# Napoliee/Expressive-FastSpeech2-Mandarin

Hardware: AMD Instinct MI355X
Metric: mel-frames/sec/GPU (batch-64 synth) at 1/2/4/8 MI355X; RTF (higher is better)
Workload: dtype bf16; 1 GPU; cfg2: batch=64 x 64 phonemes per GPU, ESD-Chinese-Singing-MFA model.yaml, FastSpeech2.forward eval bf16; global_batch=64, seq_len=64, mel_frames_per_gpu_batch=24883, T_max=430, parallelism=dp1 (independent shards, no collective), hip_graph=True

## Files before the change

### expressive-fastspeech2-mandarin_amd/csrc/lr.hip

```cpp
#include <cstdlib>
#include <type_traits>

#include "fs2_common.h"
#include "fs2hip_prosody.h"

namespace {

constexpr int kScanThreads = 256;
constexpr int kLdsCum = 2048;

__device__ __forceinline__ int64_t frames_of(const void *dur, int kind, float d_control, const float *d_map,
                                             int64_t idx, float *d_rounded) {
  if (kind == FS2_DUR_I64) {
    int64_t d = reinterpret_cast<const int64_t *>(dur)[idx];
    return d > 0 ? d : 0;
  }
  float v = reinterpret_cast<const float *>(dur)[idx];
  if (kind == FS2_DUR_LOGPRED) {
    float r = rintf(expf(v) - 1.0f) * (d_map != nullptr ? d_map[idx] : d_control);
    r = r < 0.0f ? 0.0f : r;
    if (d_rounded) d_rounded[idx] = r;
    v = r;
  }
  if (!(v > 0.0f)) return 0;
  if (v >= 9.2e18f) return INT64_MAX / 4;
  return (int64_t)v;
}

__global__ __launch_bounds__(kScanThreads) void lr_durations_kernel(const void *dur, int kind, float d_control,
                                                                    const float *d_map, int L, int32_t *cum,
                                                                    int64_t *mel_len, float *d_rounded) {
  const int b = blockIdx.x;
  const int tid = threadIdx.x;
  const int lane = tid & 63, wid = tid >> 6;
  const int per = (L + kScanThreads - 1) / kScanThreads;
  const int i0 = min(tid * per, L), i1 = min(i0 + per, L);
  const int64_t base = (int64_t)b * L;

  int64_t local = 0;
  for (int i = i0; i < i1; ++i) local += frames_of(dur, kind, d_control, d_map, base + i, nullptr);

  int64_t incl = local;
#pragma unroll
  for (int o = 1; o < 64; o <<= 1) {
    int64_t y = __shfl_up(incl, o, 64);
    if (lane >= o) incl += y;
  }
  __shared__ int64_t wave_tot[kScanThreads / 64];
  if (lane == 63) wave_tot[wid] = incl;
  __syncthreads();
  int64_t prefix = 0;
  for (int w = 0; w < wid; ++w) prefix += wave_tot[w];
  int64_t run = prefix + incl - local;

  for (int i = i0; i < i1; ++i) {
    run += frames_of(dur, kind, d_control, d_map, base + i, d_rounded);
    cum[base + i] = (int32_t)(run < 0x7fffffff ? run : 0x7fffffff);
  }
  if (tid == kScanThreads - 1) {
    int64_t total = 0;
    for (int w = 0; w < kScanThreads / 64; ++w) total += wave_tot[w];
    mel_len[b] = total;
  }
}

template <typename TX, typename TO, bool HAS_PE, int ROWS, bool NT>
__global__ __launch_bounds__(256) void lr_expand_kernel(const TX *__restrict__ x, const int32_t *__restrict__ cum,
                                                        const int64_t *__restrict__ mel_len, int L, int D, int T_out,
                                                        const float *__restrict__ pe, TO *__restrict__ out,
                                                        int32_t *__restrict__ index_map,
                                                        const int32_t *__restrict__ out_cu) {
  constexpr int UNR = ROWS / 8;
  const int b = blockIdx.y;
  const int t0 = blockIdx.x * ROWS;
  const int tid = threadIdx.x;
  const int t_end = out_cu != nullptr ? min(T_out, out_cu[b + 1] - out_cu[b]) : T_out;
  if (t0 >= t_end && index_map == nullptr) return;
  __shared__ int src[ROWS];
  __shared__ int32_t scum[kLdsCum];
  const int64_t ml = mel_len[b];
  const int lim = (int)(ml < (int64_t)T_out ? ml : (int64_t)T_out);
  const int32_t *c = cum + (int64_t)b * L;
  const bool in_lds = L <= kLdsCum;
  if (in_lds)
    for (int i = tid; i < L; i += 256) scum[i] = c[i];
  __syncthreads();
  const int32_t *sc = in_lds ? scum : c;
  if (tid < ROWS) {
    const int t = t0 + tid;
    int s = -1;
    if (t < lim) {
      int lo = 0, hi = L - 1;
      while (lo < hi) {
        const int mid = (lo + hi) >> 1;
        if (sc[mid] > t) hi = mid; else lo = mid + 1;
      }
      s = lo;
    }
    src[tid] = s;
    if (index_map != nullptr && t < T_out) index_map[(int64_t)b * T_out + t] = s;
  }
  __syncthreads();
  if (out == nullptr) return;
  const int vpr = D >> 3;
  const int rows = min(ROWS, t_end - t0);
  if (rows <= 0) return;
  const int total = rows * vpr;
  const TX *xb = x + (int64_t)b * L * D;
  TO *ob = out + ((out_cu != nullptr ? (int64_t)out_cu[b] : (int64_t)b * T_out) + t0) * D;
  for (int base = tid; base < total; base += 256 * UNR) {
    float v[UNR][8];
#pragma unroll
    for (int u = 0; u < UNR; ++u) {
      const int e = base + u * 256;
      const int r = e / vpr;
      const int col = (e - r * vpr) << 3;
      const int s = e < total ? src[r] : -1;
      if (s >= 0) {
        load8(xb + (int64_t)s * D + col, v[u]);
      } else {
#pragma unroll
        for (int q = 0; q < 8; ++q) v[u][q] = 0.0f;
      }
      if constexpr (HAS_PE) {
        if (e < total) {
          float p[8];
          load8(pe + (int64_t)(t0 + r) * D + col, p);
#pragma unroll
          for (int q = 0; q < 8; ++q) v[u][q] += p[q];
        }
      }
    }
#pragma unroll
    for (int u = 0; u < UNR; ++u) {
      const int e = base + u * 256;
      if (e < total) {
        if constexpr (NT && sizeof(TO) == 2) {
          bf16x8 o;
#pragma unroll
          for (int q = 0; q < 8; ++q) o[q] = (bf16)v[u][q];
          __builtin_nontemporal_store(o, reinterpret_cast<bf16x8 *>(ob + (int64_t)e * 8));
        } else {
          store8(ob + (int64_t)e * 8, v[u]);
        }
      }
    }
  }
}

template <typename TX, typename TO, int ROWS, bool NT>
void launch_expand_v(const void *x, const int32_t *cum, const int64_t *mel_len, int B, int L, int D, int T_out,
                     const float *pe, void *out, int32_t *index_map, const int32_t *out_cu, hipStream_t s) {
  dim3 grid((T_out + ROWS - 1) / ROWS, B);
  if (pe != nullptr)
    hipLaunchKernelGGL((lr_expand_kernel<TX, TO, true, ROWS, NT>), grid, dim3(256), 0, s,
                       reinterpret_cast<const TX *>(x), cum, mel_len, L, D, T_out, pe, reinterpret_cast<TO *>(out),
                       index_map, out_cu);
  else
    hipLaunchKernelGGL((lr_expand_kernel<TX, TO, false, ROWS, NT>), grid, dim3(256), 0, s,
                       reinterpret_cast<const TX *>(x), cum, mel_len, L, D, T_out, pe, reinterpret_cast<TO *>(out),
                       index_map, out_cu);
}

template <typename TX, typename TO>
void launch_expand(const void *x, const int32_t *cum, const int64_t *mel_len, int B, int L, int D, int T_out,
                   const float *pe, void *out, int32_t *index_map, const int32_t *out_cu, hipStream_t s) {
  launch_expand_v<TX, TO, 32, true>(x, cum, mel_len, B, L, D, T_out, pe, out, index_map, out_cu, s);
}

__global__ __launch_bounds__(256) void lr_bwd_kernel(const float *__restrict__ dy, const int32_t *__restrict__ cum,
                                                     int L, int D, int T, float *__restrict__ dx) {
  constexpr int PH = 8;
  const int b = blockIdx.y, i0 = blockIdx.x * PH;
  const int vpr = D >> 3;
  const int32_t *c = cum + (int64_t)b * L;
  const float *db = dy + (int64_t)b * T * D;
  for (int e = threadIdx.x; e < PH * vpr; e += 256) {
    const int i = i0 + e / vpr;
    if (i >= L) break;
    const int col = (e - (i - i0) * vpr) << 3;
    const int t0 = i == 0 ? 0 : min(c[i - 1], T);
    const int t1 = min(c[i], T);
    float acc[8] = {0.f, 0.f, 0.f, 0.f, 0.f, 0.f, 0.f, 0.f};
    for (int t = t0; t < t1; ++t) {
      float v[8];
      load8(db + (int64_t)t * D + col, v);
#pragma unroll
      for (int q = 0; q < 8; ++q) acc[q] += v[q];
    }
    store8(dx + ((int64_t)b * L + i) * D + col, acc);
  }
}

struct LrFusedArgs {
  const void *x;
  const void *dur;
  int dur_kind;
  float d_control;
  const float *d_map;
  const int32_t *cum_in;
  const int64_t *mel_len_in;
  const int64_t *lens;
  int B, L, D, T;
  const float *pe;
  void *out;
  int32_t *cum;
  int64_t *mel_len;
  float *d_rounded;
  int32_t *cu;
  int2 *row_pos;
  int32_t *rowmap;
  int store;
  const float *proj_src;
  const float *proj_pe;
  int NP;
  bf16 *proj_out;
  int padded;
  int32_t *index_map;
};

template <typename TX, typename TO, bool HAS_PE, int ROWS>
__global__ __launch_bounds__(256) void lr_fused_kernel(LrFusedArgs a) {
  constexpr int UNR = ROWS / 8 < 8 ? ROWS / 8 : 8;
  const int b = blockIdx.y, t0 = blockIdx.x * ROWS;
  const int tid = threadIdx.x, lane = tid & 63, wv = tid >> 6;
  const int L = a.L, T = a.T, D = a.D;
  __shared__ int32_t scum[kLdsCum];
  __shared__ int src[ROWS];
  __shared__ int64_t wtot[4];
  __shared__ int32_t wcu[4];
  __shared__ int64_t s_ml;
  const bool first = blockIdx.x == 0;
  auto clen = [&](int j) {
    const int64_t l = a.lens[j];
    return (int32_t)(l < 0 ? 0 : (l > T ? T : l));
  };
  int32_t part = 0;
  if (!a.padded)
    for (int j = tid; j < b; j += 256) part += clen(j);

  if (a.dur != nullptr) {
    const int per = (L + 255) / 256;
    const int i0 = min(tid * per, L), i1 = min(i0 + per, L);
    const int64_t base = (int64_t)b * L;
    int64_t local = 0;
    for (int i = i0; i < i1; ++i) local += frames_of(a.dur, a.dur_kind, a.d_control, a.d_map, base + i, nullptr);
    int64_t incl = local;
#pragma unroll
    for (int o = 1; o < 64; o <<= 1) {
      const int64_t y = __shfl_up(incl, o, 64);
      if (lane >= o) incl += y;
    }
    if (lane == 63) wtot[wv] = incl;
    __syncthreads();
    int64_t run = incl - local;
    for (int w = 0; w < wv; ++w) run += wtot[w];
    for (int i = i0; i < i1; ++i) {
      run += frames_of(a.dur, a.dur_kind, a.d_control, a.d_map, base + i, first ? a.d_rounded : nullptr);
      const int32_t c = (int32_t)(run < 0x7fffffff ? run : 0x7fffffff);
      scum[i] = c;
      if (first) a.cum[base + i] = c;
    }
    if (tid == 0) {
      const int64_t total = (wtot[0] + wtot[1]) + (wtot[2] + wtot[3]);
      s_ml = total;
      if (first) a.mel_len[b] = total;
    }
  } else {
    const int32_t *c = a.cum_in + (int64_t)b * L;
    for (int i = tid; i < L; i += 256) scum[i] = c[i];
    if (tid == 0) s_ml = a.mel_len_in[b];
  }

#pragma unroll
  for (int o = 32; o > 0; o >>= 1) part += __shfl_xor(part, o, 64);
  if (lane == 0) wcu[wv] = part;
  __syncthreads();
  const int32_t cu_b = a.padded ? b * T : (wcu[0] + wcu[1]) + (wcu[2] + wcu[3]);
  const int32_t len_b = a.padded ? T : clen(b);
  if (first && tid == 0 && !a.padded) {
    a.cu[b] = cu_b;
    if (b == a.B - 1) a.cu[a.B] = cu_b + len_b;
  }

  const int64_t ml = s_ml;
  const int lim = (int)(ml < (int64_t)T ? ml : (int64_t)T);
  if (tid < ROWS) {
    const int t = t0 + tid;
    int sidx = -1;
    if (t < lim) {
      int lo = 0, hi = L - 1;
      while (lo < hi) {
        const int mid = (lo + hi) >> 1;
        if (scum[mid] > t) hi = mid; else lo = mid + 1;
      }
      sidx = lo;
    }
    src[tid] = sidx;
    if (a.index_map != nullptr && t < T) a.index_map[(int64_t)b * T + t] = sidx;
    if (t < T && !a.padded) {
      if (a.rowmap != nullptr) a.rowmap[(int64_t)b * T + t] = t < len_b ? cu_b + t : -1;
      if (a.row_pos != nullptr && t < len_b) a.row_pos[cu_b + t] = make_int2(t, len_b);
    }
  }
  __syncthreads();

  const int rows = min(ROWS, min(T, (int)len_b) - t0);
  if (rows <= 0) return;
  const int vpr = D >> 3, total = rows * vpr;
  const TX *xb = reinterpret_cast<const TX *>(a.x) + (int64_t)b * L * D;
  TO *ob = reinterpret_cast<TO *>(a.out) + ((int64_t)cu_b + t0) * D;
  const bool proj = a.proj_out != nullptr;
  auto gather = [&](auto UC, int me, int nthr) {
    constexpr int U = decltype(UC)::value;
    for (int base = me; base < total; base += nthr * U) {
      float v[U][8];
#pragma unroll
      for (int u = 0; u < U; ++u) {
        const int e = base + u * nthr;
        const int r = e / vpr;
        const int col = (e - r * vpr) << 3;
        const int sidx = e < total ? src[r] : -1;
        if (sidx >= 0) {
          load8(xb + (int64_t)sidx * D + col, v[u]);
        } else {
#pragma unroll
          for (int q = 0; q < 8; ++q) v[u][q] = 0.0f;
        }
        if constexpr (HAS_PE) {
          if (e < total) {
            float pv[8];
            load8(a.pe + (int64_t)(t0 + r) * D + col, pv);
#pragma unroll
            for (int q = 0; q < 8; ++q) v[u][q] += pv[q];
          }
        }
      }
#pragma unroll
      for (int u = 0; u < U; ++u) {
        const int e = base + u * nthr;
        if (e < total) {
          if constexpr (sizeof(TO) == 2) {
            bf16x8 o;
#pragma unroll
            for (int q = 0; q < 8; ++q) o[q] = (bf16)v[u][q];
            bf16x8 *dst = reinterpret_cast<bf16x8 *>(ob + (int64_t)e * 8);
            if (a.store == 0)
              __builtin_nontemporal_store(o, dst);
            else if (a.store == 1)
              *dst = o;
            else
              __builtin_amdgcn_raw_buffer_store_b128(__builtin_bit_cast(__attribute__((ext_vector_type(4))) unsigned, o),
                                                     __builtin_amdgcn_make_buffer_rsrc(dst, (short)0, 16, 0x00020000), 0u,
                                                     0, 16);
          } else {
            store8(ob + (int64_t)e * 8, v[u]);
          }
        }
      }
    }
  };
  gather(std::integral_constant<int, UNR>{}, tid, 256);
  if (proj && wv < 3) {
    constexpr int RB = 8;
    const int NP = a.NP, cg = NP >> 3;
    const float *tb = a.proj_pe + (int64_t)t0 * NP;
    const float *sb = a.proj_src + (int64_t)b * L * NP;
    bf16 *pb = a.proj_out + ((int64_t)cu_b + t0) * NP;
    const int lanes = 192 / cg * cg;
    if (tid < lanes) {
      const int c = (tid % cg) * 8, r1 = tid / cg, rs = lanes / cg;
      for (int r0 = r1; r0 < rows; r0 += RB * rs) {
        float4 tv[RB][2], sv[RB][2];
#pragma unroll
        for (int u = 0; u < RB; ++u) {
          const int r = min(r0 + u * rs, rows - 1);
          const int sidx = src[r];
          const float *tp = tb + (int64_t)r * NP + c;
          tv[u][0] = *reinterpret_cast<const float4 *>(tp);
          tv[u][1] = *reinterpret_cast<const float4 *>(tp + 4);
          if (sidx >= 0) {
            const float *sp = sb + (int64_t)sidx * NP + c;
            sv[u][0] = *reinterpret_cast<const float4 *>(sp);
            sv[u][1] = *reinterpret_cast<const float4 *>(sp + 4);
          } else {
            sv[u][0] = sv[u][1] = make_float4(0.f, 0.f, 0.f, 0.f);
          }
        }
#pragma unroll
        for (int u = 0; u < RB; ++u) {
          const int r = r0 + u * rs;
          if (r < rows) {
            const bf16x8 o{(bf16)(tv[u][0].x + sv[u][0].x), (bf16)(tv[u][0].y + sv[u][0].y),
                           (bf16)(tv[u][0].z + sv[u][0].z), (bf16)(tv[u][0].w + sv[u][0].w),
                           (bf16)(tv[u][1].x + sv[u][1].x), (bf16)(tv[u][1].y + sv[u][1].y),
                           (bf16)(tv[u][1].z + sv[u][1].z), (bf16)(tv[u][1].w + sv[u][1].w)};
            __builtin_nontemporal_store(o, reinterpret_cast<bf16x8 *>(pb + (int64_t)r * NP + c));
          }
        }
      }
    }
  }
}

__global__ __launch_bounds__(256) void length_mask_kernel(const int64_t *__restrict__ lens, int width, int64_t n,
                                                          bool *__restrict__ mask) {
  const int64_t i = (int64_t)blockIdx.x * 256 + threadIdx.x;
  if (i >= n) return;
  const int64_t b = i / width;
  mask[i] = (int64_t)(i - b * width) >= lens[b];
}

__global__ __launch_bounds__(256) void seq_cu_kernel(const int64_t *__restrict__ lens, int B, int T,
                                                     int32_t *__restrict__ cu) {
  __shared__ int32_t part[257];
  const int tid = threadIdx.x;
  const int per = (B + 255) / 256;
  const int i0 = min(tid * per, B), i1 = min(i0 + per, B);
  int32_t local = 0;
  for (int i = i0; i < i1; ++i) {
    const int64_t l = lens[i];
    local += (int32_t)(l < 0 ? 0 : (l > T ? T : l));
  }
  part[tid + 1] = local;
  if (tid == 0) part[0] = 0;
  __syncthreads();
  if (tid == 0)
    for (int i = 1; i <= 256; ++i) part[i] += part[i - 1];
  __syncthreads();
  int32_t run = part[tid];
  for (int i = i0; i < i1; ++i) {
    cu[i] = run;
    const int64_t l = lens[i];
    run += (int32_t)(l < 0 ? 0 : (l > T ? T : l));
  }
  if (tid == 255) cu[B] = part[256];
}

__global__ __launch_bounds__(256) void seq_rows_kernel(const int32_t *__restrict__ cu, int B, int T,
                                                       int2 *__restrict__ row_pos, int32_t *__restrict__ rowmap) {
  const int64_t i = (int64_t)blockIdx.x * 256 + threadIdx.x;
  if (i >= (int64_t)B * T) return;
  const int b = (int)(i / T), t = (int)(i - (int64_t)b * T);
  const int c = cu[b], len = cu[b + 1] - c;
  if (rowmap != nullptr) rowmap[i] = t < len ? c + t : -1;
  if (row_pos != nullptr && t < len) row_pos[c + t] = make_int2(t, len);
}

constexpr int kSeqMaxB = 4096;
__global__ __launch_bounds__(256) void seq_layout_kernel(const int64_t *__restrict__ lens, int B, int T,
                                                         int32_t *__restrict__ cu, int2 *__restrict__ row_pos,
                                                         int32_t *__restrict__ rowmap, int margin) {
  __shared__ int32_t scu[kSeqMaxB + 1];
  __shared__ int32_t wsum[4];
  const int tid = threadIdx.x, lane = tid & 63, wv = tid >> 6;
  const int per = (B + 255) / 256;
  const int i0 = min(tid * per, B), i1 = min(i0 + per, B);
  auto clen = [&](int i) {
    int64_t l = lens[i];
    if (margin > 0) l = l + 2 * (int64_t)margin > T ? T : l + margin;
    return (int32_t)(l < 0 ? 0 : (l > T ? T : l));
  };
  int32_t local = 0;
  for (int i = i0; i < i1; ++i) local += clen(i);
  int32_t v = local;
#pragma unroll
  for (int o = 1; o < 64; o <<= 1) {
    const int32_t u = __shfl_up(v, o);
    if (lane >= o) v += u;
  }
  if (lane == 63) wsum[wv] = v;
  __syncthreads();
  int32_t run = v - local;
  for (int w = 0; w < wv; ++w) run += wsum[w];
  for (int i = i0; i < i1; ++i) {
    scu[i] = run;
    run += clen(i);
  }
  if (tid == 0) scu[B] = wsum[0] + wsum[1] + wsum[2] + wsum[3];
  __syncthreads();
  if (blockIdx.x == 0)
    for (int i = tid; i <= B; i += 256) cu[i] = scu[i];
  const int64_t i = (int64_t)blockIdx.x * 256 + tid;
  if (i >= (int64_t)B * T) return;
  const int b = (int)(i / T), t = (int)(i - (int64_t)b * T);
  const int c = scu[b], len = scu[b + 1] - c;
  if (rowmap != nullptr) rowmap[i] = t < len ? c + t : -1;
  if (row_pos != nullptr && t < len) row_pos[c + t] = make_int2(t, len);
}

__global__ __launch_bounds__(256) void len_stats_kernel(const int64_t *__restrict__ lens, int B,
                                                        const int32_t *__restrict__ bad, int32_t *__restrict__ meta) {
  __shared__ int64_t smax[4], ssum[4];
  const int tid = threadIdx.x, lane = tid & 63, wv = tid >> 6;
  int64_t mx = 0, sm = 0;
  for (int i = tid; i < B; i += 256) {
    const int64_t l = lens[i] < 0 ? 0 : lens[i];
    mx = l > mx ? l : mx;
    sm += l;
  }
#pragma unroll
  for (int o = 32; o > 0; o >>= 1) {
    const int64_t a = __shfl_xor(mx, o), b = __shfl_xor(sm, o);
    mx = a > mx ? a : mx;
    sm += b;
  }
  if (lane == 0) {
    smax[wv] = mx;
    ssum[wv] = sm;
  }
  __syncthreads();
  if (tid == 0) {
    int64_t m = 0, t = 0;
    for (int w = 0; w < 4; ++w) {
      m = smax[w] > m ? smax[w] : m;
      t += ssum[w];
    }
    meta[0] = (int32_t)(m < 0x7fffffff ? m : 0x7fffffff);
    meta[1] = (int32_t)(t < 0x7fffffff ? t : 0x7fffffff);
    meta[2] = bad != nullptr ? *bad : 0;
  }
}

}

extern "C" int fs2_seq_layout_margin(const int64_t *lens, int B, int T, int margin, int32_t *cu, int32_t *row_pos,
                                     int32_t *rowmap, fs2_stream_t stream) {
  if (lens == nullptr || cu == nullptr || B < 0 || T < 0 || margin < 0 || B > kSeqMaxB ||
      (int64_t)B * T > 0x7fffff00LL)
    return FS2_EINVAL;
  const int64_t n = (int64_t)B * T;
  hipLaunchKernelGGL(seq_layout_kernel, dim3((unsigned)(n > 0 ? (n + 255) / 256 : 1)), dim3(256), 0, as_stream(stream),
                     lens, B, T, cu, reinterpret_cast<int2 *>(row_pos), rowmap, margin);
  FS2_CHECK_LAUNCH();
  return FS2_OK;
}

extern "C" int fs2_seq_layout(const int64_t *lens, int B, int T, int32_t *cu, int32_t *row_pos, int32_t *rowmap,
                              fs2_stream_t stream) {
  if (lens == nullptr || cu == nullptr || B < 0 || T < 0 || (int64_t)B * T > 0x7fffff00LL) return FS2_EINVAL;
  hipStream_t s = as_stream(stream);
  if (B <= kSeqMaxB) return fs2_seq_layout_margin(lens, B, T, 0, cu, row_pos, rowmap, stream);
  hipLaunchKernelGGL(seq_cu_kernel, dim3(1), dim3(256), 0, s, lens, B, T, cu);
  FS2_CHECK_LAUNCH();
  if ((rowmap != nullptr || row_pos != nullptr) && (int64_t)B * T > 0) {
    hipLaunchKernelGGL(seq_rows_kernel, dim3((unsigned)(((int64_t)B * T + 255) / 256)), dim3(256), 0, s, cu, B, T,
                       reinterpret_cast<int2 *>(row_pos), rowmap);
    FS2_CHECK_LAUNCH();
  }
  return FS2_OK;
}

extern "C" int fs2_length_masks(const int64_t *lens, int B, int width, bool *mask, fs2_stream_t stream) {
  if (lens == nullptr || mask == nullptr || B < 0 || width < 0) return FS2_EINVAL;
  const int64_t n = (int64_t)B * width;
  if (n == 0) return FS2_OK;
  hipLaunchKernelGGL(length_mask_kernel, dim3((unsigned)((n + 255) / 256)), dim3(256), 0, as_stream(stream), lens, width,
                     n, mask);
  FS2_CHECK_LAUNCH();
  return FS2_OK;
}

extern "C" int fs2_lr_durations_map(const void *dur, int dur_kind, float d_control, const float *d_map, int B, int L,
                                    int32_t *cum, int64_t *mel_len, float *d_rounded, fs2_stream_t stream) {
  if (dur == nullptr || cum == nullptr || mel_len == nullptr || B < 0 || L <= 0) return FS2_EINVAL;
  if (dur_kind < FS2_DUR_I64 || dur_kind > FS2_DUR_LOGPRED) return FS2_EINVAL;
  if (d_map != nullptr && dur_kind != FS2_DUR_LOGPRED) return FS2_EINVAL;
  if (B == 0) return FS2_OK;
  hipLaunchKernelGGL(lr_durations_kernel, dim3(B), dim3(kScanThreads), 0, as_stream(stream), dur, dur_kind, d_control,
                     d_map, L, cum, mel_len, d_rounded);
  FS2_CHECK_LAUNCH();
  return FS2_OK;
}

extern "C" int fs2_lr_durations(const void *dur, int dur_kind, float d_control, int B, int L, int32_t *cum,
                                int64_t *mel_len, float *d_rounded, fs2_stream_t stream) {
  return fs2_lr_durations_map(dur, dur_kind, d_control, nullptr, B, L, cum, mel_len, d_rounded, stream);
}

extern "C" int fs2_lr_expand(const void *x, int x_dtype, const int32_t *cum, const int64_t *mel_len, int B, int L,
                             int D, int T_out, const float *pe, void *out, int out_dtype, int32_t *index_map,
                             const int32_t *out_cu, fs2_stream_t stream) {
  if (x == nullptr || cum == nullptr || mel_len == nullptr || (out == nullptr && index_map == nullptr))
    return FS2_EINVAL;
  if (B < 0 || L <= 0 || D <= 0 || (D & 7) != 0 || T_out < 0) return FS2_EINVAL;
  if (B == 0 || T_out == 0) return FS2_OK;
  hipStream_t s = as_stream(stream);
  if (x_dtype == FS2_F32 && out_dtype == FS2_F32)
    launch_expand<float, float>(x, cum, mel_len, B, L, D, T_out, pe, out, index_map, out_cu, s);
  else if (x_dtype == FS2_BF16 && out_dtype == FS2_BF16)
    launch_expand<bf16, bf16>(x, cum, mel_len, B, L, D, T_out, pe, out, index_map, out_cu, s);
  else if (x_dtype == FS2_F32 && out_dtype == FS2_BF16)
    launch_expand<float, bf16>(x, cum, mel_len, B, L, D, T_out, pe, out, index_map, out_cu, s);
  else if (x_dtype == FS2_BF16 && out_dtype == FS2_F32)
    launch_expand<bf16, float>(x, cum, mel_len, B, L, D, T_out, pe, out, index_map, out_cu, s);
  else
    return FS2_EUNSUPPORTED;
  FS2_CHECK_LAUNCH();
  return FS2_OK;
}

static int lr_fused_launch(const LrFusedArgs &a, int x_dtype, int out_dtype, hipStream_t s);

template <typename TX, typename TO, bool HAS_PE, int FR>
__global__ __launch_bounds__(256) void lr_pad_kernel(LrFusedArgs a) {
  constexpr int PER = 4;
  constexpr int U = 8;
  const int b = blockIdx.y, t0 = blockIdx.x * FR;
  const int tid = threadIdx.x, lane = tid & 63, wv = tid >> 6;
  const int L = a.L, T = a.T, D = a.D;
  __shared__ int src[FR];
  __shared__ int64_t wtot[4];
  const bool first = blockIdx.x == 0;
  if (tid < FR) src[tid] = -1;
  const int per = (L + 255) >> 8;
  const int i0 = min(tid * per, L), i1 = min(i0 + per, L);
  const int64_t base = (int64_t)b * L;
  int64_t fr[PER];
  int64_t local = 0;
#pragma unroll
  for (int k = 0; k < PER; ++k) {
    fr[k] = i0 + k < i1 ? frames_of(a.dur, a.dur_kind, a.d_control, a.d_map, base + i0 + k,
                                    first ? a.d_rounded : nullptr)
                        : 0;
    local += fr[k];
  }
  int64_t incl = local;
#pragma unroll
  for (int o = 1; o < 64; o <<= 1) {
    const int64_t y = __shfl_up(incl, o, 64);
    if (lane >= o) incl += y;
  }
  if (lane == 63) wtot[wv] = incl;
  __syncthreads();
  int64_t run = incl - local;
  for (int w = 0; w < wv; ++w) run += wtot[w];
  const int64_t f0 = t0, f1 = min(t0 + FR, T);
#pragma unroll
  for (int k = 0; k < PER; ++k) {
    if (i0 + k < i1) {
      const int64_t s = run;
      run += fr[k];
      if (first) a.cum[base + i0 + k] = (int32_t)(run < 0x7fffffff ? run : 0x7fffffff);
      const int lo = (int)(s > f0 ? s : f0), hi = (int)(run < f1 ? run : f1);
      for (int t = lo; t < hi; ++t) src[t - t0] = i0 + k;
    }
  }
  if (first && tid == 0) a.mel_len[b] = (wtot[0] + wtot[1]) + (wtot[2] + wtot[3]);
  __syncthreads();
  if (a.index_map != nullptr && tid < FR && t0 + tid < T) a.index_map[(int64_t)b * T + t0 + tid] = src[tid];

  const int rows = min(FR, T - t0);
  const int vpr = D >> 3, total = rows * vpr;
  const TX *xb = reinterpret_cast<const TX *>(a.x) + base * D;
  TO *ob = reinterpret_cast<TO *>(a.out) + ((int64_t)b * T + t0) * D;
  for (int e0 = tid; e0 < total; e0 += 256 * U) {
    float v[U][8];
#pragma unroll
    for (int u = 0; u < U; ++u) {
      const int e = e0 + u * 256;
      const int r = e / vpr, col = (e - r * vpr) << 3;
      const int s = e < total ? src[r] : -1;
      if (s >= 0) {
        load8(xb + (int64_t)s * D + col, v[u]);
      } else {
#pragma unroll
        for (int q = 0; q < 8; ++q) v[u][q] = 0.0f;
      }
      if constexpr (HAS_PE) {
        if (e < total) {
          float pv[8];
          load8(a.pe + (int64_t)(t0 + r) * D + col, pv);
#pragma unroll
          for (int q = 0; q < 8; ++q) v[u][q] += pv[q];
        }
      }
    }
#pragma unroll
    for (int u = 0; u < U; ++u) {
      const int e = e0 + u * 256;
      if (e < total) {
        if constexpr (sizeof(TO) == 2) {
          bf16x8 o;
#pragma unroll
          for (int q = 0; q < 8; ++q) o[q] = (bf16)v[u][q];
          __builtin_nontemporal_store(o, reinterpret_cast<bf16x8 *>(ob + (int64_t)e * 8));
        } else {
          store8(ob + (int64_t)e * 8, v[u]);
        }
      }
    }
  }
}

template <typename TX, typename TO>
static void lr_pad_launch(const LrFusedArgs &a, int fr, hipStream_t s) {
  const dim3 grid((unsigned)((a.T + fr - 1) / fr), (unsigned)a.B);
  auto go = [&](auto FRC) {
    constexpr int F = decltype(FRC)::value;
    if (a.pe != nullptr)
      hipLaunchKernelGGL((lr_pad_kernel<TX, TO, true, F>), grid, dim3(256), 0, s, a);
    else
      hipLaunchKernelGGL((lr_pad_kernel<TX, TO, false, F>), grid, dim3(256), 0, s, a);
  };
  if (fr == 256)
    go(std::integral_constant<int, 256>{});
  else if (fr == 128)
    go(std::integral_constant<int, 128>{});
  else
    go(std::integral_constant<int, 64>{});
}

extern "C" int fs2_length_regulate(const void *x, int x_dtype, const void *dur, int dur_kind, float d_control, int B,
                                   int L, int D, int T_out, const float *pe, void *out, int out_dtype, int32_t *cum,
                                   int64_t *mel_len, float *d_rounded, int32_t *index_map, fs2_stream_t stream) {
  return fs2_length_regulate_map(x, x_dtype, dur, dur_kind, d_control, nullptr, B, L, D, T_out, pe, out, out_dtype, cum,
                                 mel_len, d_rounded, index_map, stream);
}

extern "C" int fs2_length_regulate_map(const void *x, int x_dtype, const void *dur, int dur_kind, float d_control,
                                       const float *d_map, int B, int L, int D, int T_out, const float *pe, void *out,
                                       int out_dtype, int32_t *cum, int64_t *mel_len, float *d_rounded,
                                       int32_t *index_map, fs2_stream_t stream) {
  if (x == nullptr || dur == nullptr || cum == nullptr || mel_len == nullptr) return FS2_EINVAL;
  if (dur_kind < FS2_DUR_I64 || dur_kind > FS2_DUR_LOGPRED) return FS2_EINVAL;
  if (d_map != nullptr && dur_kind != FS2_DUR_LOGPRED) return FS2_EINVAL;
  if (dur_kind == FS2_DUR_LOGPRED && d_rounded == nullptr) return FS2_EINVAL;
  if (out == nullptr && index_map == nullptr) return FS2_EINVAL;
  if (B < 0 || L <= 0 || D <= 0 || (D & 7) != 0 || T_out < 0 || (int64_t)B * T_out > 0x7fffff00LL) return FS2_EINVAL;
  if (B == 0) return FS2_OK;
  if (T_out == 0 || L > kLdsCum || out == nullptr) {
    const int rc = fs2_lr_durations_map(dur, dur_kind, d_control, d_map, B, L, cum, mel_len, d_rounded, stream);
    if (rc != FS2_OK || T_out == 0) return rc;
    return fs2_lr_expand(x, x_dtype, cum, mel_len, B, L, D, T_out, pe, out, out_dtype, index_map, nullptr, stream);
  }
  LrFusedArgs a{};
  a.x = x;
  a.dur = dur;
  a.dur_kind = dur_kind;
  a.d_control = d_control;
  a.d_map = d_map;
  a.B = B;
  a.L = L;
  a.D = D;
  a.T = T_out;
  a.pe = pe;
  a.out = out;
  a.cum = cum;
  a.mel_len = mel_len;
  a.d_rounded = d_rounded;
  a.padded = 1;
  a.index_map = index_map;
  if (L > 1024) return lr_fused_launch(a, x_dtype, out_dtype, as_stream(stream));
  static const int fr_env = [] {
    const char *e = getenv("FS2_LR_PAD_FR");
    const int v = e != nullptr ? atoi(e) : 0;
    return (v == 64 || v == 128 || v == 256) ? v : 0;
  }();
  const int fr = fr_env != 0 ? fr_env : (int64_t)B * ((T_out + 127) / 128) >= 512 ? 128 : 64;
  hipStream_t s = as_stream(stream);
  if (x_dtype == FS2_BF16 && out_dtype == FS2_BF16)
    lr_pad_launch<bf16, bf16>(a, fr, s);
  else if (x_dtype == FS2_F32 && out_dtype == FS2_F32)
    lr_pad_launch<float, float>(a, fr, s);
  else if (x_dtype == FS2_F32 && out_dtype == FS2_BF16)
    lr_pad_launch<float, bf16>(a, fr, s);
  else if (x_dtype == FS2_BF16 && out_dtype == FS2_F32)
    lr_pad_launch<bf16, float>(a, fr, s);
  else
    return FS2_EUNSUPPORTED;
  FS2_CHECK_LAUNCH();
  return FS2_OK;
}

extern "C" int fs2_lr_backward(const float *dy, const int32_t *cum, int B, int L, int D, int T, float *dx,
                               fs2_stream_t stream) {
  if (dy == nullptr || cum == nullptr || dx == nullptr || B < 0 || L < 0 || T < 0 || D <= 0 || (D & 7) || D > 2048)
    return FS2_EINVAL;
  if (B == 0 || L == 0) return FS2_OK;
  hipLaunchKernelGGL(lr_bwd_kernel, dim3((unsigned)((L + 7) / 8), (unsigned)B), dim3(256), 0, as_stream(stream), dy,
                     cum, L, D, T, dx);
  FS2_CHECK_LAUNCH();
  return FS2_OK;
}

extern "C" int fs2_len_stats(const int64_t *lens, int B, const int32_t *bad_counter, int32_t *meta, fs2_stream_t stream) {
  if (lens == nullptr || meta == nullptr || B < 0) return FS2_EINVAL;
  hipLaunchKernelGGL(len_stats_kernel, dim3(1), dim3(256), 0, as_stream(stream), lens, B, bad_counter, meta);
  FS2_CHECK_LAUNCH();
  return FS2_OK;
}

extern "C" int fs2_lr_fused(const void *x, int x_dtype, const void *dur, int dur_kind, float d_control,
                            const int32_t *cum_in, const int64_t *mel_len_in, int B, int L, int D, int T_out,
                            const float *pe, const int64_t *layout_lens, int32_t *cu, int32_t *row_pos,
                            int32_t *rowmap, void *out, int out_dtype, int32_t *cum, int64_t *mel_len,
                            float *d_rounded, fs2_stream_t stream) {
  return fs2_lr_fused_proj(x, x_dtype, dur, dur_kind, d_control, cum_in, mel_len_in, B, L, D, T_out, pe, layout_lens,
                           cu, row_pos, rowmap, out, out_dtype, cum, mel_len, d_rounded, nullptr, nullptr, 0, nullptr,
                           stream);
}

extern "C" int fs2_lr_fused_proj(const void *x, int x_dtype, const void *dur, int dur_kind, float d_control,
                                 const int32_t *cum_in, const int64_t *mel_len_in, int B, int L, int D, int T_out,
                                 const float *pe, const int64_t *layout_lens, int32_t *cu, int32_t *row_pos,
                                 int32_t *rowmap, void *out, int out_dtype, int32_t *cum, int64_t *mel_len,
                                 float *d_rounded, const float *proj_src, const float *proj_pe, int NP,
                                 void *proj_out, fs2_stream_t stream) {
  return fs2_lr_fused_proj_map(x, x_dtype, dur, dur_kind, d_control, nullptr, cum_in, mel_len_in, B, L, D, T_out, pe,
                               layout_lens, cu, row_pos, rowmap, out, out_dtype, cum, mel_len, d_rounded, proj_src,
                               proj_pe, NP, proj_out, stream);
}

extern "C" int fs2_lr_fused_proj_map(const void *x, int x_dtype, const void *dur, int dur_kind, float d_control,
                                     const float *d_map, const int32_t *cum_in, const int64_t *mel_len_in, int B,
                                     int L, int D, int T_out, const float *pe, const int64_t *layout_lens, int32_t *cu,
                                     int32_t *row_pos, int32_t *rowmap, void *out, int out_dtype, int32_t *cum,
                                     int64_t *mel_len, float *d_rounded, const float *proj_src, const float *proj_pe,
                                     int NP, void *proj_out, fs2_stream_t stream) {
  if (d_map != nullptr && (dur == nullptr || dur_kind != FS2_DUR_LOGPRED)) return FS2_EINVAL;
  if (proj_out != nullptr && (proj_src == nullptr || proj_pe == nullptr || NP < 8 || NP > 1536 || (NP & 7) != 0))
    return FS2_EINVAL;
  if (x == nullptr || out == nullptr || layout_lens == nullptr || cu == nullptr) return FS2_EINVAL;
  if (B < 0 || L <= 0 || D <= 0 || (D & 7) != 0 || T_out < 0 || B > kSeqMaxB || L > kLdsCum) return FS2_EINVAL;
  if ((int64_t)B * T_out > 0x7fffff00LL) return FS2_EINVAL;
  if (dur != nullptr) {
    if (cum == nullptr || mel_len == nullptr || dur_kind < FS2_DUR_I64 || dur_kind > FS2_DUR_LOGPRED) return FS2_EINVAL;
    if (dur_kind == FS2_DUR_LOGPRED && d_rounded == nullptr) return FS2_EINVAL;
  } else if (cum_in == nullptr || mel_len_in == nullptr) {
    return FS2_EINVAL;
  }
  if (B == 0) return FS2_OK;
  if (T_out == 0) {
    if (dur != nullptr) {
      int rc = fs2_lr_durations_map(dur, dur_kind, d_control, d_map, B, L, cum, mel_len, d_rounded, stream);
      if (rc != FS2_OK) return rc;
    }
    return fs2_seq_layout(layout_lens, B, 0, cu, row_pos, rowmap, stream);
  }
  LrFusedArgs a{};
  a.x = x;
  a.dur = dur;
  a.dur_kind = dur_kind;
  a.d_control = d_control;
  a.d_map = d_map;
  a.cum_in = cum_in;
  a.mel_len_in = mel_len_in;
  a.lens = layout_lens;
  a.B = B;
  a.L = L;
  a.D = D;
  a.T = T_out;
  a.pe = pe;
  a.out = out;
  a.cum = cum;
  a.mel_len = mel_len;
  a.d_rounded = d_rounded;
  a.cu = cu;
  a.row_pos = reinterpret_cast<int2 *>(row_pos);
  a.rowmap = rowmap;
  static const int store_env = [] {
    const char *e = getenv("FS2_LR_STORE");
    return e == nullptr ? 0 : (e[0] == 'p' ? 1 : e[0] == 's' ? 2 : 0);
  }();
  a.store = store_env;
  a.proj_src = proj_src;
  a.proj_pe = proj_pe;
  a.NP = NP;
  a.proj_out = reinterpret_cast<bf16 *>(proj_out);
  return lr_fused_launch(a, x_dtype, out_dtype, as_stream(stream));
}

static int lr_fused_launch(const LrFusedArgs &a, int x_dtype, int out_dtype, hipStream_t s) {
  const int T_out = a.T, B = a.B;
  static const int rows_env = [] {
    const char *e = getenv("FS2_LR_ROWS");
    const int v = e != nullptr ? atoi(e) : 32;
    return (v == 64 || v == 128) ? v : 32;
  }();
  const int R = rows_env;
  const dim3 grid((unsigned)((T_out + R - 1) / R), (unsigned)B);
  auto go = [&](auto TXv, auto TOv) {
    using TX = decltype(TXv);
    using TO = decltype(TOv);
    auto launch = [&](auto RC) {
      constexpr int RR = decltype(RC)::value;
      if (a.pe != nullptr)
        hipLaunchKernelGGL((lr_fused_kernel<TX, TO, true, RR>), grid, dim3(256), 0, s, a);
      else
        hipLaunchKernelGGL((lr_fused_kernel<TX, TO, false, RR>), grid, dim3(256), 0, s, a);
    };
    if (R == 128)
      launch(std::integral_constant<int, 128>{});
    else if (R == 64)
      launch(std::integral_constant<int, 64>{});
    else
      launch(std::integral_constant<int, 32>{});
  };
  if (x_dtype == FS2_BF16 && out_dtype == FS2_BF16)
    go(bf16{}, bf16{});
  else if (x_dtype == FS2_F32 && out_dtype == FS2_F32)
    go(0.0f, 0.0f);
  else if (x_dtype == FS2_F32 && out_dtype == FS2_BF16)
    go(0.0f, bf16{});
  else if (x_dtype == FS2_BF16 && out_dtype == FS2_F32)
    go(bf16{}, 0.0f);
  else
    return FS2_EUNSUPPORTED;
  FS2_CHECK_LAUNCH();
  return FS2_OK;
}
```

Before: 19.17 million mel-frames/s.

## Add frame-major length-regulator kernel grouping utterances per block

Adds a new length-regulator kernel that tiles by frame chunk (FR frames) across a group of 8 utterances. Each block loads the positional-encoding and projected-PE rows once and reuses them for all 8 utterances. Row gathers are software-pipelined with a register double/quad buffer, and the per-block duration scan and cu prefix are recomputed in-kernel. It is selected by default when shapes match (D=256, NP=768, L<=256, bf16 out, unpadded). The cost is redundant per-block scans and prefix sums, plus higher register pressure.

```diff
diff --git a/expressive-fastspeech2-mandarin_amd/csrc/lr.hip b/expressive-fastspeech2-mandarin_amd/csrc/lr.hip
--- a/expressive-fastspeech2-mandarin_amd/csrc/lr.hip
+++ b/expressive-fastspeech2-mandarin_amd/csrc/lr.hip
@@ -400,6 +400,211 @@
         }
       }
     }
+  }
+}
+
+constexpr int kFmUG = 8;
+constexpr int kFmL = 256;
+constexpr int kFmD = 256, kFmNP = 768;
+
+template <typename TX, int FR>
+__global__ __launch_bounds__(256) void lr_frame_major_kernel(LrFusedArgs a) {
+  constexpr int UG = kFmUG, VPR = kFmD / 8, CG = kFmNP / 8;
+  constexpr int XP = FR * VPR / 256, PP = FR * CG / 256;
+  constexpr int DEPTH = FR <= 8 ? 4 : 2;
+  static_assert(FR * VPR % 256 == 0 && FR * CG % 256 == 0 && DEPTH <= UG && UG <= 64, "whole pieces per thread");
+  const int t0 = blockIdx.x * FR, b0 = blockIdx.y * UG;
+  const int tid = threadIdx.x, lane = tid & 63, wv = tid >> 6;
+  const int L = a.L, T = a.T, B = a.B;
+  __shared__ int32_t scum[UG][kFmL];
+  __shared__ int src[UG][FR];
+  __shared__ int32_t wcu[4];
+  __shared__ int32_t s_cu[UG], s_len[UG];
+  __shared__ int s_lim[UG];
+  const bool first = blockIdx.x == 0;
+  auto clen = [&](int j) {
+    const int64_t l = a.lens[j];
+    return (int32_t)(l < 0 ? 0 : (l > T ? T : l));
+  };
+  int32_t part = 0;
+  for (int j = tid; j < b0; j += 256) part += clen(j);
+  const int32_t len_l = wv == 0 && lane < UG && b0 + lane < B ? clen(b0 + lane) : 0;
+
+  float pv[XP][8];
+  float4 tv[PP][2];
+#pragma unroll
+  for (int k = 0; k < XP; ++k) {
+    const int e = tid + k * 256, r = e / VPR, col = (e - r * VPR) << 3;
+    load8(a.pe + (int64_t)min(t0 + r, T - 1) * kFmD + col, pv[k]);
+  }
+#pragma unroll
+  for (int k = 0; k < PP; ++k) {
+    const int e = tid + k * 256, r = e / CG, c = (e - r * CG) << 3;
+    const float *tp = a.proj_pe + (int64_t)min(t0 + r, T - 1) * kFmNP + c;
+    tv[k][0] = *reinterpret_cast<const float4 *>(tp);
+    tv[k][1] = *reinterpret_cast<const float4 *>(tp + 4);
+  }
+
+  for (int u = wv; u < UG; u += 4) {
+    const int b = b0 + u;
+    if (b >= B) continue;
+    const int64_t base = (int64_t)b * L;
+    int64_t ml;
+    if (a.dur != nullptr) {
+      const int per = (L + 63) >> 6;
+      const int i0 = min(lane * per, L), i1 = min(i0 + per, L);
+      int64_t fr[4];
+      int64_t local = 0;
+#pragma unroll
+      for (int k = 0; k < 4; ++k) {
+        fr[k] = i0 + k < i1 ? frames_of(a.dur, a.dur_kind, a.d_control, a.d_map, base + i0 + k,
+                                        first ? a.d_rounded : nullptr)
+                            : 0;
+        local += fr[k];
+      }
+      int64_t incl = local;
+#pragma unroll
+      for (int o = 1; o < 64; o <<= 1) {
+        const int64_t y = __shfl_up(incl, o, 64);
+        if (lane >= o) incl += y;
+      }
+      int64_t run = incl - local;
+#pragma unroll
+      for (int k = 0; k < 4; ++k) {
+        if (i0 + k < i1) {
+          run += fr[k];
+          const int32_t c = (int32_t)(run < 0x7fffffff ? run : 0x7fffffff);
+          scum[u][i0 + k] = c;
+          if (first) a.cum[base + i0 + k] = c;
+        }
+      }
+      ml = __shfl(incl, 63, 64);
+      if (first && lane == 0) a.mel_len[b] = ml;
+    } else {
+      for (int i = lane; i < L; i += 64) scum[u][i] = a.cum_in[base + i];
+      ml = a.mel_len_in[b];
+    }
+    if (lane == 0) s_lim[u] = (int)(ml < (int64_t)T ? ml : (int64_t)T);
+  }
+
+#pragma unroll
+  for (int o = 32; o > 0; o >>= 1) part += __shfl_xor(part, o, 64);
+  if (lane == 0) wcu[wv] = part;
+  __syncthreads();
+  if (wv == 0) {
+    const int b = b0 + lane;
+    const int32_t len = len_l;
+    int32_t incl = len;
+#pragma unroll
+    for (int o = 1; o < UG; o <<= 1) {
+      const int32_t y = __shfl_up(incl, o, 64);
+      if (lane >= o) incl += y;
+    }
+    const int32_t cu_b = (wcu[0] + wcu[1]) + (wcu[2] + wcu[3]) + incl - len;
+    if (lane < UG) {
+      s_cu[lane] = cu_b;
+      s_len[lane] = len;
+      if (first && b < B) {
+        a.cu[b] = cu_b;
+        if (b == B - 1) a.cu[B] = cu_b + len;
+      }
+    }
+  }
+  __syncthreads();
+
+  for (int p = tid; p < UG * FR; p += 256) {
+    const int u = p / FR, r = p - u * FR, b = b0 + u, t = t0 + r;
+    if (b >= B) continue;
+    int sidx = -1;
+    if (t < s_lim[u]) {
+      int lo = 0, hi = L - 1;
+      while (lo < hi) {
+        const int mid = (lo + hi) >> 1;
+        if (scum[u][mid] > t) hi = mid; else lo = mid + 1;
+      }
+      sidx = lo;
+    }
+    src[u][r] = sidx;
+    if (t < T) {
+      const int32_t cu_b = s_cu[u], len_b = s_len[u];
+      if (a.rowmap != nullptr) a.rowmap[(int64_t)b * T + t] = t < len_b ? cu_b + t : -1;
+      if (a.row_pos != nullptr && t < len_b) a.row_pos[cu_b + t] = make_int2(t, len_b);
+    }
+  }
+  __syncthreads();
+
+  auto rows_of = [&](int u) {
+    return __builtin_amdgcn_readfirstlane(b0 + u < B ? min(FR, min(T, (int)s_len[u]) - t0) : 0);
+  };
+  auto fetch = [&](int u, float(&xv)[XP][8], float4(&sv)[PP][2]) {
+    unsigned keep = 0;
+    const int rows = rows_of(u);
+    if (rows <= 0) return keep;
+    const int64_t base = (int64_t)(b0 + u) * L;
+#pragma unroll
+    for (int k = 0; k < XP; ++k) {
+      const int e = tid + k * 256, r = e / VPR, col = (e - r * VPR) << 3;
+      const int sidx = r < rows ? src[u][r] : -1;
+      keep |= (sidx >= 0 ? 1u : 0u) << k;
+      load8(reinterpret_cast<const TX *>(a.x) + (base + max(sidx, 0)) * kFmD + col, xv[k]);
+    }
+#pragma unroll
+    for (int k = 0; k < PP; ++k) {
+      const int e = tid + k * 256, r = e / CG, c = (e - r * CG) << 3;
+      const int sidx = r < rows ? src[u][r] : -1;
+      keep |= (sidx >= 0 ? 1u : 0u) << (XP + k);
+      const float *sp = a.proj_src + (base + max(sidx, 0)) * kFmNP + c;
+      sv[k][0] = *reinterpret_cast<const float4 *>(sp);
+      sv[k][1] = *reinterpret_cast<const float4 *>(sp + 4);
+    }
+    return keep;
+  };
+  auto emit = [&](int u, unsigned keep, float(&xv)[XP][8], float4(&sv)[PP][2]) {
+    const int rows = rows_of(u);
+    if (rows <= 0) return;
+    const int64_t row0 = (int64_t)s_cu[u] + t0;
+    bf16 *ob = reinterpret_cast<bf16 *>(a.out) + row0 * kFmD;
+    bf16 *pb = a.proj_out + row0 * kFmNP;
+#pragma unroll
+    for (int k = 0; k < XP; ++k) {
+      const int e = tid + k * 256;
+      const bool kp = (keep >> k) & 1u;
+      bf16x8 o;
+#pragma unroll
+      for (int q = 0; q < 8; ++q) o[q] = (bf16)((kp ? xv[k][q] : 0.0f) + pv[k][q]);
+      if (e < rows * VPR) {
+        bf16x8 *dst = reinterpret_cast<bf16x8 *>(ob + (int64_t)e * 8);
+        if (a.store == 0)
+          __builtin_nontemporal_store(o, dst);
+        else if (a.store == 1)
+          *dst = o;
+        else
+          __builtin_amdgcn_raw_buffer_store_b128(__builtin_bit_cast(__attribute__((ext_vector_type(4))) unsigned, o),
+                                                 __builtin_amdgcn_make_buffer_rsrc(dst, (short)0, 16, 0x00020000), 0u,
+                                                 0, 16);
+      }
+    }
+#pragma unroll
+    for (int k = 0; k < PP; ++k) {
+      const int e = tid + k * 256;
+      const bool kp = (keep >> (XP + k)) & 1u;
+      const float4 s0 = kp ? sv[k][0] : make_float4(0.f, 0.f, 0.f, 0.f);
+      const float4 s1 = kp ? sv[k][1] : make_float4(0.f, 0.f, 0.f, 0.f);
+      const bf16x8 o{(bf16)(tv[k][0].x + s0.x), (bf16)(tv[k][0].y + s0.y), (bf16)(tv[k][0].z + s0.z),
+                     (bf16)(tv[k][0].w + s0.w), (bf16)(tv[k][1].x + s1.x), (bf16)(tv[k][1].y + s1.y),
+                     (bf16)(tv[k][1].z + s1.z), (bf16)(tv[k][1].w + s1.w)};
+      if (e < rows * CG) __builtin_nontemporal_store(o, reinterpret_cast<bf16x8 *>(pb + (int64_t)e * 8));
+    }
+  };
+  float xs[DEPTH][XP][8];
+  float4 ss[DEPTH][PP][2];
+  unsigned ks[DEPTH];
+#pragma unroll
+  for (int u = 0; u < DEPTH - 1; ++u) ks[u] = fetch(u, xs[u], ss[u]);
+#pragma unroll
+  for (int u = 0; u < UG; ++u) {
+    if (u + DEPTH - 1 < UG) ks[(u + DEPTH - 1) % DEPTH] = fetch(u + DEPTH - 1, xs[(u + DEPTH - 1) % DEPTH], ss[(u + DEPTH - 1) % DEPTH]);
+    emit(u, ks[u % DEPTH], xs[u % DEPTH], ss[u % DEPTH]);
   }
 }
 
@@ -871,8 +1076,34 @@
   return lr_fused_launch(a, x_dtype, out_dtype, as_stream(stream));
 }
 
+static bool lr_frame_major_ok(const LrFusedArgs &a, int out_dtype) {
+  const char *e = getenv("FS2_LR_FORM");
+  if (e != nullptr && e[0] == '0') return false;
+  return !a.padded && a.index_map == nullptr && a.proj_out != nullptr && a.pe != nullptr && out_dtype == FS2_BF16 &&
+         a.D == kFmD && a.NP == kFmNP && a.L <= kFmL;
+}
+
+template <typename TX>
+static void lr_frame_major_launch(const LrFusedArgs &a, hipStream_t s) {
+  const char *e = getenv("FS2_LR_FR");
+  const int fr = e != nullptr && atoi(e) == 16 ? 16 : 8;
+  const dim3 grid((unsigned)((a.T + fr - 1) / fr), (unsigned)((a.B + kFmUG - 1) / kFmUG));
+  if (fr == 8)
+    hipLaunchKernelGGL((lr_frame_major_kernel<TX, 8>), grid, dim3(256), 0, s, a);
+  else
+    hipLaunchKernelGGL((lr_frame_major_kernel<TX, 16>), grid, dim3(256), 0, s, a);
+}
+
 static int lr_fused_launch(const LrFusedArgs &a, int x_dtype, int out_dtype, hipStream_t s) {
   const int T_out = a.T, B = a.B;
+  if (lr_frame_major_ok(a, out_dtype) && (x_dtype == FS2_BF16 || x_dtype == FS2_F32)) {
+    if (x_dtype == FS2_BF16)
+      lr_frame_major_launch<bf16>(a, s);
+    else
+      lr_frame_major_launch<float>(a, s);
+    FS2_CHECK_LAUNCH();
+    return FS2_OK;
+  }
   static const int rows_env = [] {
     const char *e = getenv("FS2_LR_ROWS");
     const int v = e != nullptr ? atoi(e) : 32;
```

Measured after the change: 19.12 million mel-frames/s. No clear change (-0.3%).
